# MiksuNy/rust_ray_tracing

Measured on AMD Instinct MI355X. Metric: Mray/s at 1920x1080, 8 spp, Sponza BVH; 1/2/4/8-GPU scaling + % HBM roofline, higher is better.
Workload: dtype f32

## Files before the change

include/mipt_diag.h:

```cpp
#ifndef MIPT_DIAG_H
#define MIPT_DIAG_H

#include <stdint.h>

#ifdef __cplusplus
extern "C" {
#endif

#if defined(__GNUC__)
#define MIPT_DIAG_API __attribute__((visibility("default")))
#else
#define MIPT_DIAG_API
#endif

MIPT_DIAG_API int mipt_debug_eval(int op, const float *a, const float *b, uint64_t n, float *out);

MIPT_DIAG_API int mipt_debug_eval_range(int op, uint32_t first_bits, uint64_t n, float y, float *out);

MIPT_DIAG_API int mipt_debug_wgsl(int op, const float *in, uint64_t n, const uint32_t *texels, uint32_t tex_w, uint32_t tex_h, float *out);

MIPT_DIAG_API int mipt_debug_divide(float *d_buf, uint64_t n_floats, float divisor, void *stream);
MIPT_DIAG_API int mipt_debug_popcount(const uint32_t *d_bitmap, uint64_t n_words, uint64_t *d_out, void *stream);

MIPT_DIAG_API const char *mipt_diag_last_error(void);

MIPT_DIAG_API int mipt_internal_pair_order(const void *nodes, uint32_t n_nodes, uint32_t *order_out, uint32_t cap, uint32_t *n_records_out);
MIPT_DIAG_API uint32_t mipt_internal_pair_order_top(void);
MIPT_DIAG_API int mipt_internal_tri_slots(const void *nodes, uint32_t n_nodes, uint32_t n_tris, uint32_t *slot_out, uint32_t *n_slots_out);

MIPT_DIAG_API int mipt_diag_scene_sizes(const void *scene, uint64_t out[2]);
MIPT_DIAG_API int mipt_diag_scene_read(const void *scene, int which, void *dst, uint64_t bytes);
MIPT_DIAG_API int mipt_diag_scene_hash(const void *scene, uint64_t out[2]);

MIPT_DIAG_API int mipt_diag_host_layout(const void *desc, uint8_t *geom_out, uint64_t geom_cap, uint8_t *attr_out, uint64_t attr_cap,
                                        uint64_t *sizes_out, uint32_t *info_out);

MIPT_DIAG_API int mipt_diag_hash_words(const void *words, uint64_t n_words, uint64_t *out);

MIPT_DIAG_API int mipt_diag_write_obj(const char *path, const void *tris, uint64_t n_tris, const char *mtllib, const char *const *material_names,
                                      uint32_t n_materials);

#ifdef __cplusplus
}
#endif
#endif
```

rust_ray_tracing_amd/_lib.py:

```python
from __future__ import annotations

import ctypes as C
import os

import numpy as np

_HERE = os.path.dirname(os.path.abspath(__file__))
LIB_PATH = os.environ.get("MIPT_LIB") or os.path.join(_HERE, "libmipt.so")

VERTEX = np.dtype([("position", "<f4", 3), ("tex_coord_x", "<f4"), ("normal", "<f4", 3), ("tex_coord_y", "<f4")])
TRIANGLE = np.dtype([("vertices", VERTEX, 3), ("material_id", "<u4"), ("_pad", "u1", 12)])
NODE = np.dtype([("bounds_min", "<f4", 3), ("first_tri_or_child", "<u4"), ("bounds_max", "<f4", 3), ("num_tris", "<u4")])
MATERIAL = np.dtype([
    ("base_color", "<f4", 3), ("transmission", "<f4"), ("specular_tint", "<f4", 3), ("ior", "<f4"),
    ("emission", "<f4", 3), ("roughness", "<f4"), ("metallic", "<f4"), ("transparency", "<f4"),
    ("base_color_tex_id", "<u4"), ("transparency_tex_id", "<u4"), ("roughness_tex_id", "<u4"),
    ("metallic_tex_id", "<u4"), ("emission_tex_id", "<u4"), ("normal_tex_id", "<u4")])
CAMERA = np.dtype([("look_at", "<f4", (4, 4)), ("position", "<f4", 3), ("_pad", "<f4")])
assert VERTEX.itemsize == 32 and TRIANGLE.itemsize == 112 and NODE.itemsize == 32
assert MATERIAL.itemsize == 80 and CAMERA.itemsize == 80

NO_TEXTURE = 0xFFFFFFFF

SEED_PIXEL_STREAM, SEED_PER_SAMPLE = 0, 1
# ... 240 lines not shown
    lib.mipt_query_closest_device.argtypes = [vp, vp, u64, qo, vp, vp, C.POINTER(MiptStats)]
    lib.mipt_query_closest_device.restype = C.c_int
    lib.mipt_query_occluded.argtypes = [vp, vp, u64, qo, vp, C.POINTER(MiptStats)]
    lib.mipt_query_occluded.restype = C.c_int
    lib.mipt_query_occluded_device.argtypes = [vp, vp, u64, qo, vp, vp, C.POINTER(MiptStats)]
    lib.mipt_query_occluded_device.restype = C.c_int
    fb = C.POINTER(MiptFeatureBuffers)
    lib.mipt_render_features.argtypes = [vp, vp, u32, C.POINTER(MiptOptions), fb, C.POINTER(MiptStats)]
    lib.mipt_render_features.restype = C.c_int
    lib.mipt_render_features_device.argtypes = [vp, vp, u32, C.POINTER(MiptOptions), fb, vp, C.POINTER(MiptStats)]
    lib.mipt_render_features_device.restype = C.c_int
    return lib


MULTITEST_LIB_PATH = os.path.join(_HERE, "libmipt_multitest.so")
_multitest = None


def load_multitest() -> C.CDLL:
    global _multitest
    if _multitest is not None:
        return _multitest
    load()
    if not os.path.exists(MULTITEST_LIB_PATH):
        raise ImportError(f"{MULTITEST_LIB_PATH} is missing: run __graft_entry__.build()")
    lib = _bind(C.CDLL(MULTITEST_LIB_PATH))
    lib.rccl_double_inject.argtypes = [C.c_int, C.c_int]
    lib.rccl_double_inject.restype = C.c_longlong
    _multitest = lib
    return lib


DIAG_LIB_PATH = os.path.join(_HERE, "libmipt_diag.so")
DIAG_EXPORTS = ["mipt_debug_eval", "mipt_debug_eval_range", "mipt_debug_wgsl", "mipt_debug_divide", "mipt_debug_popcount", "mipt_diag_last_error",
                "mipt_internal_pair_order", "mipt_internal_pair_order_top", "mipt_internal_tri_slots",
                "mipt_diag_scene_sizes", "mipt_diag_scene_read", "mipt_diag_scene_hash", "mipt_diag_write_obj", "mipt_diag_host_layout", "mipt_diag_hash_words"]
_diag = None


def load_diag() -> C.CDLL:
    global _diag
    if _diag is not None:
        return _diag
    load()
    if not os.path.exists(DIAG_LIB_PATH):
        raise ImportError(f"{DIAG_LIB_PATH} is missing: run __graft_entry__.build()")
    lib = C.CDLL(DIAG_LIB_PATH)
    vp = C.c_void_p
    lib.mipt_debug_eval.argtypes = [C.c_int, vp, vp, C.c_uint64, vp]
    lib.mipt_debug_eval.restype = C.c_int
    lib.mipt_debug_eval_range.argtypes = [C.c_int, C.c_uint32, C.c_uint64, C.c_float, vp]
    lib.mipt_debug_eval_range.restype = C.c_int
    lib.mipt_debug_wgsl.argtypes = [C.c_int, vp, C.c_uint64, vp, C.c_uint32, C.c_uint32, vp]
    lib.mipt_debug_wgsl.restype = C.c_int
    lib.mipt_debug_divide.argtypes = [vp, C.c_uint64, C.c_float, vp]
    lib.mipt_debug_divide.restype = C.c_int
    lib.mipt_debug_popcount.argtypes = [vp, C.c_uint64, vp, vp]
    lib.mipt_debug_popcount.restype = C.c_int
    lib.mipt_diag_last_error.argtypes = []
    lib.mipt_diag_last_error.restype = C.c_char_p
    u32p = C.POINTER(C.c_uint32)
    lib.mipt_internal_pair_order.argtypes = [vp, C.c_uint32, vp, C.c_uint32, u32p]
    lib.mipt_internal_pair_order.restype = C.c_int
    lib.mipt_internal_pair_order_top.argtypes = []
    lib.mipt_internal_pair_order_top.restype = C.c_uint32
    lib.mipt_internal_tri_slots.argtypes = [vp, C.c_uint32, C.c_uint32, vp, u32p]
    lib.mipt_internal_tri_slots.restype = C.c_int
    lib.mipt_diag_scene_sizes.argtypes = [vp, C.POINTER(C.c_uint64 * 2)]
    lib.mipt_diag_scene_sizes.restype = C.c_int
    lib.mipt_diag_scene_read.argtypes = [vp, C.c_int, vp, C.c_uint64]
    lib.mipt_diag_scene_read.restype = C.c_int
    lib.mipt_diag_scene_hash.argtypes = [vp, C.POINTER(C.c_uint64 * 2)]
    lib.mipt_diag_scene_hash.restype = C.c_int
    lib.mipt_diag_write_obj.argtypes = [C.c_char_p, vp, C.c_uint64, C.c_char_p, C.POINTER(C.c_char_p), C.c_uint32]
    lib.mipt_diag_write_obj.restype = C.c_int
    lib.mipt_diag_host_layout.argtypes = [vp, vp, C.c_uint64, vp, C.c_uint64, C.POINTER(C.c_uint64 * 2), C.POINTER(C.c_uint32 * 4)]
    lib.mipt_diag_host_layout.restype = C.c_int
    lib.mipt_diag_hash_words.argtypes = [vp, C.c_uint64, C.POINTER(C.c_uint64)]
    lib.mipt_diag_hash_words.restype = C.c_int
    _diag = lib
    return lib


class MiptError(RuntimeError):
    def __init__(self, code: int, where: str):
        self.code = code
        msg = load().mipt_last_error()
        super().__init__(f"{where} failed with status {code}: {msg.decode() if msg else ''}")


def check(code: int, where: str) -> None:
# ... 7 lines not shown
```

rust_ray_tracing_amd/csrc/mipt_api.cpp:

```cpp
#include "../../include/mipt.h"
#include "pt_kernel.h"
#include "mipt_scene.h"

#include <atomic>
#include <chrono>
#include <cmath>
#include <cstdarg>
#include <cstdio>
#include <cstdlib>
#include <cstring>
#include <exception>
#include <memory>
#include <mutex>
#include <new>
#include <string>
#include <thread>
#include <vector>

static_assert(sizeof(MiptVec3) == 12, "Vec3f");
static_assert(sizeof(MiptVertex) == 32, "Vertex");
static_assert(sizeof(MiptTriangle) == 112 && offsetof(MiptTriangle, material_id) == 96, "Triangle");
static_assert(sizeof(MiptNode) == 32 && offsetof(MiptNode, first_tri_or_child) == 12 &&
                  offsetof(MiptNode, bounds_max) == 16 && offsetof(MiptNode, num_tris) == 28, "Node");
static_assert(sizeof(MiptMaterial) == 80 && offsetof(MiptMaterial, ior) == 28 && offsetof(MiptMaterial, emission) == 32 &&
                  offsetof(MiptMaterial, roughness) == 44 && offsetof(MiptMaterial, base_color_tex_id) == 56, "Material");
static_assert(sizeof(MiptCamera) == 80 && offsetof(MiptCamera, position) == 64, "UniformCamera");
static_assert(sizeof(MiptStats) == 8 + 22 * 8 && sizeof(MiptOptions) == 64, "ABI struct sizes (tests/test_abi.py, rust_ray_tracing_amd/_lib.py)");
static_assert(sizeof(MiptSceneInfo) == 64, "MiptSceneInfo");
static_assert(sizeof(mipt::DevMaterial) == 64 && sizeof(mipt::DevMaterialFull) == 128, "device records");

namespace {

thread_local std::string g_err;

}

void mipt_internal_set_error(const char *msg) { g_err = msg ? msg : ""; }

void mipt::free_scene(MiptScene *s) {
    if (!s) return;
    (void)hipSetDevice(s->device);
    mipt::free_mesh(s);
    void *ptrs[] = {s->d_geom, s->d_tri_attr, s->d_mats, s->d_mats_full, s->d_texels, s->d_nodes, s->d_tri_order,
                    s->d_stats, s->d_ovf, s->d_hdr, s->d_rgba, s->d_touched, s->d_refit_plan, s->d_refit_pair, s->d_cams, s->d_qrays, s->d_qout};
    for (void *p : ptrs)
        if (p) (void)hipFree(p);
    if (s->ev0) (void)hipEventDestroy(s->ev0);
    if (s->ev1) (void)hipEventDestroy(s->ev1);
    delete s;
}

namespace {

using mipt::fail;
using mipt::free_scene;

double now_ms() { return std::chrono::duration<double, std::milli>(std::chrono::steady_clock::now().time_since_epoch()).count(); }

template <class T>
int upload(void **dst, const T *src, size_t count, size_t min_bytes = 16) {
    size_t bytes = count * sizeof(T);
    size_t alloc = bytes < min_bytes ? min_bytes : bytes;
    MIPT_HIP(hipMalloc(dst, alloc));
    if (bytes) MIPT_HIP(hipMemcpy(*dst, src, bytes, hipMemcpyHostToDevice));
    return MIPT_OK;
}
template <class T>
int upload(void **dst, const std::vector<T> &src, size_t min_bytes = 16) { return upload(dst, src.data(), src.size(), min_bytes); }

template <class F> void parallel_for(size_t n, F body) {
    unsigned t = std::thread::hardware_concurrency();
    if (t > 16u) t = 16u;
    if (t < 2u || n < (size_t)1 << 16) { body((size_t)0, n); return; }
    const size_t per = (n + t - 1) / t;
    std::vector<std::thread> th;
    size_t b = per;
    try {
// ... 423 lines not shown
    pr.samples_f = (float)opt->samples;
    pr.cull_scale = 1.0f + opt->cull_margin;
    pr.service_num = 3; pr.service_den = 8; pr.reverse_tiles = 0;
    for (int c = 0; c < 3; c++)
        for (int r = 0; r < 3; r++) pr.cam[c * 3 + r] = camera->look_at[c][r];
    pr.cam[9] = camera->position.x; pr.cam[10] = camera->position.y; pr.cam[11] = camera->position.z;
    pr.hdr = d_hdr_rgb;
    pr.stats = scene->d_stats;

    const bool count = (opt->flags & MIPT_FLAG_COUNT) != 0;
    const bool cull = opt->traversal == MIPT_TRAVERSAL_CULLED;
    const int occ = mipt::trace_blocks_per_cu(batch, count, cull, (int)opt->shading);
    int bpc = occ;
    {
        const long long fit = (long long)(pr.total_work / (unsigned long long)(1.25 * scene->n_cu * mipt::kBlockThreads));
        const int cap = (int)(fit < 2 ? 2 : fit);
        if (cap < bpc) bpc = cap;
    }
    pr.leaf_period = (pr.total_work >= 4ull * (unsigned long long)scene->n_cu * (unsigned long long)occ * mipt::kBlockThreads) ? 4u : 1u;
    pr.leaf_den = 4u;
    int grid = 0;
    if ((rc = mipt::traversal_grid(scene, bpc, pr.total_work, &grid))) return rc;
    pr.ovf = scene->d_ovf;

    const bool touched = count && (opt->flags & MIPT_FLAG_TOUCHED) != 0 && opt->shading == 0;
    const size_t geom_lines = ((size_t)scene->dev.geom_bytes + 127) / 128, attr_lines = (scene->n_tris + 1) / 2;
    const size_t geom_words = (geom_lines + 31) / 32, attr_words = (attr_lines + 31) / 32;
    pr.touched = nullptr; pr.touched_attr_base = (uint32_t)(geom_words * 32);
    if (touched) {
        if (!scene->d_touched) MIPT_HIP(hipMalloc((void **)&scene->d_touched, (geom_words + attr_words) * sizeof(uint32_t)));
        MIPT_HIP(hipMemsetAsync(scene->d_touched, 0, (geom_words + attr_words) * sizeof(uint32_t), stream));
        pr.touched = scene->d_touched;
    }
    mipt::DevBatch bt{};
    if (batch) {
        scene->h_cams.assign((size_t)n_views * 4, make_float4(0.0f, 0.0f, 0.0f, 0.0f));
        for (uint32_t v = 0; v < n_views; v++) {
            const MiptCamera &c = cameras[v];
            for (int col = 0; col < 3; col++) scene->h_cams[(size_t)v * 4 + col] = make_float4(c.look_at[col][0], c.look_at[col][1], c.look_at[col][2], 0.0f);
            scene->h_cams[(size_t)v * 4 + 3] = make_float4(c.position.x, c.position.y, c.position.z, 0.0f);
        }
        const size_t bytes = scene->h_cams.size() * sizeof(float4);
        if ((rc = mipt::grow_device_buffer((void **)&scene->d_cams, &scene->cams_bytes, bytes))) return rc;
        MIPT_HIP(hipMemcpyAsync(scene->d_cams, scene->h_cams.data(), bytes, hipMemcpyHostToDevice, stream));
        bt.cams = scene->d_cams;
        bt.view_pixels = opt->width * opt->height;
        bt.tiles_recip = 0xffffffffu / pr.n_local_tiles;
    }
    mipt::DevStats hs;
    float ms = 0.0f;
    rc = mipt::traversal_launch(
        scene, stream,
        [&]() -> int {
            MIPT_HIP(mipt::launch_trace(scene->dev, pr, batch ? &bt : nullptr, count, cull, (int)opt->shading, (int)grid, stream));
            return MIPT_OK;
        },
        [&]() -> int {
            if (touched) {
                MIPT_HIP(mipt::launch_popcount(scene->d_touched, geom_words, &scene->d_stats->touched_geom, stream));
                MIPT_HIP(mipt::launch_popcount(scene->d_touched + geom_words, attr_words, &scene->d_stats->touched_attr, stream));
            }
            if (d_rgba8) MIPT_HIP(mipt::launch_tonemap(d_hdr_rgb, (unsigned long long)opt->width * opt->height * n_views, 1.0f, d_rgba8, stream));
            return MIPT_OK;
        },
        hs, ms);
    if (rc && rc != MIPT_ERR_STACK) return rc;
    if (stats) {
        memset(stats, 0, sizeof *stats);
        stats->kernel_ms = ms;
        stats->rays = hs.rays; stats->inner_steps = hs.inner_steps; stats->tri_tests = hs.tri_tests;
        stats->hits = hs.hits; stats->texel_fetches = hs.texel_fetches; stats->stack_overflows = hs.stack_overflows;
        stats->tex_clamped = hs.tex_clamped; stats->max_stack = hs.max_stack; stats->pixels = hs.pixels;
        stats->diag[0] = hs.d_iters; stats->diag[1] = hs.d_inner_lanes; stats->diag[2] = hs.d_leaf_lanes;
        stats->diag[3] = hs.d_iters_inner; stats->diag[4] = hs.d_iters_leaf; stats->diag[5] = hs.d_services;
        stats->diag[6] = hs.d_service_lanes; stats->diag[7] = hs.d_cycles_service; stats->diag[8] = hs.d_cycles_total; stats->diag[9] = hs.d_cycles_mem; stats->diag[10] = hs.d_cycles_tail;
        stats->touched_lines[0] = hs.touched_geom; stats->touched_lines[1] = hs.touched_attr;
    }
    return rc;
}

int mipt::render_device_impl(MiptScene *scene, const MiptCamera *camera, const MiptOptions *opt,
                             float *d_hdr_rgb, uint8_t *d_rgba8, void *hip_stream, MiptStats *stats, bool pack_single) {
    return render_launch(scene, camera, 1u, false, opt, d_hdr_rgb, d_rgba8, hip_stream, stats, pack_single);
}

extern "C" {

int mipt_render_batch_device(MiptScene *scene, const MiptCamera *cameras, uint32_t n_views, const MiptOptions *opt,
                             float *d_hdr_rgb, uint8_t *d_rgba8, void *hip_stream, MiptStats *stats) {
    MIPT_NO_THROW(render_launch(scene, cameras, n_views, true, opt, d_hdr_rgb, d_rgba8, hip_stream, stats, false))
// ... 102 lines not shown
```

rust_ray_tracing_amd/csrc/mipt_diag.hip:

```cpp
#include "../../include/mipt_diag.h"
#include "pt_device_math.h"
#include "pt_device_wgsl.h"
#include "mipt_host_util.h"
#include "pt_kernel.h"

#include <stdio.h>

namespace {

thread_local char g_err[256] = "";

__global__ void debug_eval_kernel(int op, const float *__restrict__ a, const float *__restrict__ b, float b_scalar,
                                  unsigned long long n, float *__restrict__ out) {
    using namespace mipt;
    for (unsigned long long i = (unsigned long long)blockIdx.x * blockDim.x + threadIdx.x; i < n;
         i += (unsigned long long)gridDim.x * blockDim.x) {
        const float x = a[i], y = b ? b[i] : b_scalar;
        float r = 0.0f;
        switch (op) {
        case 0: r = gl_cosf(x); break;
        case 1: r = gl_log10f(x, GlTabGlobal()); break;
        case 2: r = gl_powf(x, y); break;
        case 3: r = x / y; break;
        case 4: r = __builtin_sqrtf(x); break;
        case 5: r = x * y; break;
        case 6: r = x + y; break;
        case 7: r = fminf(x, y); break;
        case 8: r = fmaxf(x, y); break;
        case 9: { uint32_t s = __float_as_uint(x); r = rand_f32(s); } break;
        case 10: { uint32_t s = __float_as_uint(x); r = rand_f32_nd(s, GlTabGlobal()); } break;
        case 11: { uint32_t s = __float_as_uint(x); V3 v = rand_in_unit_sphere(s, GlTabGlobal()); r = (y == 0.0f) ? v.x : (y == 1.0f ? v.y : v.z); } break;
        case 12: r = __uint_as_float(srgb_quantize(x)); break;
        case 13: r = x - truncf(x); break;
        case 14: r = fdiv_ray(x, y, 1.0f / y); break;
        case 15: r = u8_over_255(__float_as_uint(x)); break;
        case 16: r = gl_sinf(x); break;
        case 17: r = gl_expf(x); break;
// ... 111 lines not shown
        snprintf(g_err, sizeof g_err, "mipt_debug_wgsl: bad argument");
        return -1;
    }
    const uint64_t in_bytes = n * kWgslIn[op] * 4, out_bytes = n * kWgslOut[op] * 4;
    mipt::DevPtr<char> din, dtex, dout;
    hipError_t e;
    if ((e = din.alloc(in_bytes)) != hipSuccess) return fail(e, "hipMalloc");
    if ((e = dout.alloc(out_bytes)) != hipSuccess) return fail(e, "hipMalloc");
    if ((e = hipMemcpy(din, in, in_bytes, hipMemcpyHostToDevice)) != hipSuccess) return fail(e, "hipMemcpy");
    if (op == 0) {
        const uint64_t tex_bytes = (uint64_t)tex_w * tex_h * 4;
        if ((e = dtex.alloc(tex_bytes)) != hipSuccess) return fail(e, "hipMalloc");
        if ((e = hipMemcpy(dtex, texels, tex_bytes, hipMemcpyHostToDevice)) != hipSuccess) return fail(e, "hipMemcpy");
    }
    hipLaunchKernelGGL(debug_wgsl_kernel, dim3(1024), dim3(256), 0, nullptr, op, (const float *)din.get(), (unsigned long long)n,
                       (const uint32_t *)dtex.get(), tex_w, tex_h, (float *)dout.get(), kWgslIn[op], kWgslOut[op]);
    if ((e = hipGetLastError()) != hipSuccess) return fail(e, "launch");
    if ((e = hipMemcpy(out, dout, out_bytes, hipMemcpyDeviceToHost)) != hipSuccess) return fail(e, "hipMemcpy");
    return 0;
}

int mipt_debug_divide(float *d_buf, uint64_t n_floats, float divisor, void *stream) {
    if (!d_buf || n_floats == 0) { snprintf(g_err, sizeof g_err, "mipt_debug_divide: bad argument"); return -1; }
    const hipError_t e = mipt::launch_divide(d_buf, (unsigned long long)n_floats, divisor, (hipStream_t)stream);
    return e == hipSuccess ? 0 : fail(e, "launch_divide");
}

int mipt_debug_popcount(const uint32_t *d_bitmap, uint64_t n_words, uint64_t *d_out, void *stream) {
    if (!d_bitmap || !d_out || n_words == 0) { snprintf(g_err, sizeof g_err, "mipt_debug_popcount: bad argument"); return -1; }
    const hipError_t e = mipt::launch_popcount(d_bitmap, (unsigned long long)n_words, (unsigned long long *)d_out, (hipStream_t)stream);
    return e == hipSuccess ? 0 : fail(e, "launch_popcount");
}

const char *mipt_diag_last_error(void) { return g_err; }

}
```

rust_ray_tracing_amd/csrc/mipt_scene.h:

```cpp
#pragma once
#include "../../include/mipt.h"
#include "mipt_host_util.h"
#include "pt_kernel.h"

#include <stddef.h>

#include <memory>
#include <vector>

namespace mipt { struct SceneMesh; }

struct MiptScene {
    int device = 0;
    mipt::DevScene dev{};
    void *d_geom = nullptr, *d_tri_attr = nullptr, *d_mats = nullptr, *d_mats_full = nullptr, *d_texels = nullptr;
    size_t geom_alloc = 0, attr_bytes = 0, mats_bytes = 0, mats_full_bytes = 0, texel_bytes = 0;
    MiptNode *d_nodes = nullptr;
    uint32_t n_nodes = 0;
    uint32_t *d_tri_order = nullptr;
    MiptSceneInfo info{};
    mipt::DevStats *d_stats = nullptr;
    uint32_t *d_ovf = nullptr;
    size_t ovf_waves = 0;
    uint32_t *d_touched = nullptr;
    size_t n_tris = 0;
    float *d_hdr = nullptr;
    size_t hdr_bytes = 0;
    uint8_t *d_rgba = nullptr;
    size_t rgba_bytes = 0;
    float4 *d_cams = nullptr;
    size_t cams_bytes = 0;
    std::vector<float4> h_cams;
    void *d_qrays = nullptr, *d_qout = nullptr;
    size_t qrays_bytes = 0, qout_bytes = 0;
    hipEvent_t ev0 = nullptr, ev1 = nullptr;
    int n_cu = 0;
    uint32_t max_leaf = 0;
    uint32_t *d_refit_plan = nullptr, *d_refit_pair = nullptr;
    std::vector<uint32_t> refit_level_off;
    mipt::SceneMesh *mesh = nullptr;
};

namespace mipt {

void free_scene(MiptScene *s);
struct SceneDeleter { void operator()(MiptScene *s) const { free_scene(s); } };
using ScenePtr = std::unique_ptr<MiptScene, SceneDeleter>;
void free_mesh(MiptScene *s);
int scene_finish_workspace(MiptScene *s);
int scene_clone_to(const MiptScene *src, int device, MiptScene **out);
int scene_clone_many(const MiptScene *src, const int *device_ids, int n_dev, MiptScene **outs);

struct MaterialTables {
    std::vector<DevMaterial> mats;
    std::vector<DevMaterialFull> mats_full;
    std::vector<uint32_t> texels;
    std::vector<uint32_t> tex_offset;
    uint64_t n_texels = 0;
};
int build_material_tables(const MiptSceneDesc *desc, MaterialTables *out, bool gather_texels = true);
int upload_material_tables(MiptScene *s, const MaterialTables &t);

struct ResidentBvh {
    DevPtr<MiptNode> d_nodes;
    uint32_t n_nodes = 0;
// ... 57 lines not shown
```

rust_ray_tracing_amd/csrc/pt_kernel.h:

```cpp
#pragma once
#include <hip/hip_runtime.h>
#include <stdint.h>

namespace mipt {

struct DevMaterial {
    float base[3]; uint32_t base_off;
    float emis[3]; uint32_t emis_off;
    uint32_t base_w, base_h, emis_w, emis_h;
    uint32_t pad[4];
};

struct DevMaterialFull {
    float base[3]; float transmission;
    float emission[3]; float ior;
    float roughness, metallic, transparency, pad0;
    uint32_t tex[6][3];
    uint32_t pad1[2];
};

struct DevScene {
    const float4 *pairs;
    const float4 *tri_pos;
    uint32_t tri_off_bytes, geom_bytes;
// ... 2 lines not shown
    const DevMaterial *mats;
    const DevMaterialFull *mats_full;
    const uint32_t *texels;
    uint32_t n_pairs, n_tris, n_mats, n_texs;
    uint32_t root_a, root_n;
};

struct DevStats {
    unsigned long long queue;
    unsigned long long rays, inner_steps, tri_tests, hits, texel_fetches;
    unsigned long long stack_overflows, tex_clamped, max_stack, pixels;
    unsigned long long d_iters, d_inner_lanes, d_leaf_lanes, d_iters_inner, d_iters_leaf, d_services, d_service_lanes;
    unsigned long long d_cycles_service, d_cycles_total, d_cycles_mem, d_cycles_tail;
    unsigned long long touched_geom, touched_attr;
};

struct DevParams {
    uint32_t width, height, samples, max_depth;
    uint32_t seed_mode, sample_begin, sum_only, packed;
    uint32_t accumulate, pad1;
    uint32_t tile_rank, tile_world, tiles_x, tiles_y;
    uint32_t n_local_tiles, pad0;
    unsigned long long total_work;
    float aspect;
    float samples_f;
    float cull_scale;
    uint32_t reverse_tiles;
    uint32_t service_num, service_den;
    uint32_t leaf_period, leaf_den;
    float cam[12];
    float *hdr;
    uint32_t *ovf;
    DevStats *stats;
    uint32_t *touched;
    uint32_t touched_attr_base;
};

struct DevBatch {
    const float4 *cams;
    uint32_t view_pixels;
    uint32_t tiles_recip;
};

constexpr int kStackLds = 16;
constexpr int kStackOvf = 48;
constexpr int kWavesPerBlock = 4;
constexpr uint32_t kTriPosStride = 64;
constexpr int kBlockThreads = 64 * kWavesPerBlock;
constexpr uint32_t kMaxTris = 1u << 25;
constexpr uint32_t kMaxPairs = 1u << 24;

hipError_t launch_trace(const DevScene &sc, const DevParams &pr, const DevBatch *batch, bool count, bool cull, int shading,
                        int grid_blocks, hipStream_t stream);
int trace_blocks_per_cu(bool batch, bool count, bool cull, int shading);
hipError_t launch_unpack_tiles(const float *packed_all, uint32_t width, uint32_t height,
                               uint32_t tile_world, float *hdr, hipStream_t stream);
hipError_t launch_tonemap(const float *hdr, unsigned long long n_pixels, float divisor,
                          uint8_t *rgba8, hipStream_t stream);

struct DevQuery {
    const float4 *rays;
    void *out;
    const uint32_t *tri_order;
    unsigned long long n_rays;
    float cull_scale;
    uint32_t *ovf;
    DevStats *stats;
};
hipError_t launch_ray_query(const DevScene &sc, const DevQuery &q, bool count, bool cull, bool anyhit, int grid_blocks, hipStream_t stream);
int query_blocks_per_cu(bool count, bool cull, bool anyhit);

struct DevFeatures {
    const float4 *cams;
    float *depth; uint32_t *prim; uint32_t *material; float *position; float *uv; float *normal; float *albedo; float *emission;
    const uint32_t *tri_order;
    uint32_t width, height, samples, seed_mode;
    uint32_t sample_begin;
    uint32_t tiles_x, n_tiles;
    uint32_t tiles_recip;
    uint32_t view_pixels;
    unsigned long long total_work;
    float aspect;
    float samples_f;
    float cull_scale;
    uint32_t *ovf;
    DevStats *stats;
};
hipError_t launch_first_hit(const DevScene &sc, const DevFeatures &f, bool count, bool cull, int grid_blocks, hipStream_t stream);
int first_hit_blocks_per_cu(bool count, bool cull);

hipError_t launch_popcount(const uint32_t *bitmap, unsigned long long n_words, unsigned long long *out, hipStream_t stream);
hipError_t launch_divide(float *hdr, unsigned long long n_floats, float divisor, hipStream_t stream);
hipError_t launch_postprocess(const float *hdr, unsigned long long n_pixels, float divisor, uint16_t *rgba16,
                              hipStream_t stream);

}
```

rust_ray_tracing_amd/csrc/pt_kernel.hip:

```cpp
#include "pt_kernel.h"
#include "pt_device_math.h"
#include "pt_device_wgsl.h"
#include "pt_traverse.h"

namespace mipt {

namespace {

#ifndef MIPT_DIAG_STAMPS
#define MIPT_DIAG_STAMPS 0
#endif
constexpr bool DIAG_STAMPS = MIPT_DIAG_STAMPS != 0;

enum : uint32_t {
    ST_T = 0,
    ST_S = 1,
    ST_G = 2,
    ST_P = 3,
    ST_X = 4
};

__device__ __forceinline__ float min3_abs(float a, float b, float c) { float r; asm("v_min3_f32 %0, |%1|, |%2|, |%3|" : "=v"(r) : "v"(a), "v"(b), "v"(c)); return r; }

__device__ __forceinline__ void mark_line(uint32_t *bitmap, uint32_t line) {
// ... 210 lines not shown
                }
            }
            if (SHADING == 0) {
                float *dr = s_draw[wib];
                const unsigned long long m_sc = __ballot(scatter);
                const uint32_t n_items = 3u * (uint32_t)__popcll(m_sc);
                if (n_items != 0u) {
                    const uint32_t base = 6u * lane_rank(m_sc);
                    if (scatter) {
#pragma unroll
                        for (int k = 0; k < 6; k++) dr[base + k] = rand_f32(rng);
                    }
                    __builtin_amdgcn_fence(__ATOMIC_ACQ_REL, "wavefront");
                    __builtin_amdgcn_wave_barrier();
                    for (uint32_t item = lane; item < n_items; item += 64u) {
                        const float2 uu = *reinterpret_cast<const float2 *>(dr + 2u * item);
                        dr[2u * item] = rand_f32_nd_eval(uu.x, uu.y, (const double *)s_logtab);
                    }
                    __builtin_amdgcn_fence(__ATOMIC_ACQ_REL, "wavefront");
                    __builtin_amdgcn_wave_barrier();
                    if (scatter) {
                        const V3 rs = normalized(mk(dr[base], dr[base + 2u], dr[base + 4u]));
                        const V3 point = o + d * best_t;
                        const V3 new_dir = normalized(sc_normal + rs);
                        o = point + new_dir * 0.0001f;
                        d = new_dir;
                        bounces += 1;
                        path_done = !(bounces < pr.max_depth);
                    }
                }
            }
            if (state == ST_S) {
                if (path_done) {
                    const V3 res = (bounces == 0u) ? incoming : incoming / (float)bounces;
                    final_color = final_color + res;
                    sample += 1;
                    if (sample < pr.samples) {
                        state = ST_G;
                    } else {
                        if (!pr.sum_only) final_color = final_color / pr.samples_f;
                        float *dst = pr.hdr + (BATCH ? (size_t)view * bt.view_pixels + pix : (size_t)slot) * 3;
                        if (pr.accumulate) {
                            final_color = mk(dst[0] + final_color.x, dst[1] + final_color.y, dst[2] + final_color.z);
                        }
                        dst[0] = final_color.x; dst[1] = final_color.y; dst[2] = final_color.z;
                        c_pixels++;
                        state = ST_P;
                    }
                } else {
                    state = ST_T;
                    start_ray = true;
                }
            }
            {
                const unsigned long long m_p = __ballot(state == ST_P);
                if (m_p != 0ull) {
                    unsigned long long base = 0;
                    const uint32_t leader = (uint32_t)__ffsll((long long)m_p) - 1u;
                    if (lane == leader) base = atomicAdd(&pr.stats->queue, (unsigned long long)__popcll(m_p));
                    base = __shfl(base, (int)leader);
                    if (state == ST_P) {
                        const unsigned long long wi = base + lane_rank(m_p);
                        if (wi >= pr.total_work) {
                            state = ST_X;
                            if (COUNT && g_t_first_x == 0) g_t_first_x = clock64();
                        } else {
                            uint32_t lt = (uint32_t)(wi >> 6);
                            const uint32_t p = (uint32_t)wi & 63u;
                            if (BATCH) {
                                const uint32_t n = pr.n_local_tiles;
                                uint32_t q = __umulhi(lt, bt.tiles_recip), r = lt - q * n;
                                if (r >= n) { q += 1u; r -= n; }
                                if (r >= n) { q += 1u; r -= n; }
                                view = q; lt = r;
                            }
                            const uint32_t lt_o = pr.reverse_tiles ? (pr.n_local_tiles - 1u - lt) : lt;
                            const uint32_t gt = lt_o * pr.tile_world + pr.tile_rank;
                            const uint32_t px = (gt % pr.tiles_x) * 8u + (p & 7u);
                            const uint32_t py = (gt / pr.tiles_x) * 8u + (p >> 3);
                            if (px < pr.width && py < pr.height) {
                                pix = py * pr.width + px;
                                if (!BATCH) slot = pr.packed ? (lt_o * 64u + p) : pix;
                                rng = 987612486u * (pix + 87636354u);
                                const uint32_t y = pr.height - py;
                                screen_x = ((((float)px / (float)pr.width) * 2.0f) - 1.0f) * pr.aspect;
                                screen_y = (((float)y / (float)pr.height) * 2.0f) - 1.0f;
                                final_color = mk(0.0f, 0.0f, 0.0f);
                                sample = 0;
                                state = ST_G;
                            }
                        }
                    }
                }
            }
            if (state == ST_G) {
                if (SHADING == 1 || pr.seed_mode != 0u) {
                    const uint32_t px = pix % pr.width, py = pix / pr.width;
                    rng = (pr.sample_begin + sample) * 6023u + (757283u * px + 872653746u * py);
                }
                const float jx = (rand_f32(rng) * 2.0f - 1.0f) * 0.0005f;
                const float jy = (rand_f32(rng) * 2.0f - 1.0f) * 0.0005f;
                const float rx = -screen_x + jx, ry = screen_y + jy, rz = 1.0f;
                if (BATCH) {
                    const float4 *cr = bt.cams + (size_t)view * 4;
                    const float4 c0 = cr[0], c1 = cr[1], c2 = cr[2], c3 = cr[3];
                    const V3 dir = mk(c0.x * rx + c1.x * ry + c2.x * rz,
                                      c0.y * rx + c1.y * ry + c2.y * rz,
                                      c0.z * rx + c1.z * ry + c2.z * rz);
                    d = normalized(dir);
                    o = mk(c3.x, c3.y, c3.z);
                } else {
                    const V3 dir = mk(pr.cam[0] * rx + pr.cam[3] * ry + pr.cam[6] * rz,
                                      pr.cam[1] * rx + pr.cam[4] * ry + pr.cam[7] * rz,
                                      pr.cam[2] * rx + pr.cam[5] * ry + pr.cam[8] * rz);
                    d = normalized(dir);
// ... 138 lines not shown
        }
        {
            const unsigned long long tx = __shfl(g_t_first_x, (int)(__ffsll((long long)__ballot(g_t_first_x != 0)) - 1));
            if (lane == 0 && tx != 0) atomicAdd(&pr.stats->d_cycles_tail, clock64() - tx);
        }
    }
    if (c_pixels) atomicAdd(&pr.stats->pixels, (unsigned long long)c_pixels);
}

template <bool COUNT, bool CULL, int SHADING>
__global__ MIPT_TRACE_BOUNDS(COUNT, CULL, SHADING) void pt_trace_kernel(DevScene sc, DevParams pr) {
    trace_body<COUNT, CULL, SHADING, false>(sc, pr, DevBatch{});
}
template <bool COUNT, bool CULL, int SHADING>
__global__ MIPT_TRACE_BOUNDS(COUNT, CULL, SHADING) void pt_trace_batch_kernel(DevScene sc, DevParams pr, DevBatch bt) {
    trace_body<COUNT, CULL, SHADING, true>(sc, pr, bt);
}

__global__ void unpack_tiles_kernel(const float *__restrict__ packed_all, uint32_t width, uint32_t height,
                                    uint32_t world, uint32_t tiles_x, uint32_t n_local_tiles, float *__restrict__ hdr) {
    const unsigned long long n = (unsigned long long)width * height;
    for (unsigned long long i = (unsigned long long)blockIdx.x * blockDim.x + threadIdx.x; i < n;
         i += (unsigned long long)gridDim.x * blockDim.x) {
        const uint32_t px = (uint32_t)(i % width), py = (uint32_t)(i / width);
        const uint32_t gt = (py >> 3) * tiles_x + (px >> 3);
        const uint32_t rank = gt % world, lt = gt / world;
        const unsigned long long src = ((unsigned long long)rank * n_local_tiles + lt) * 64ull + ((py & 7u) * 8u + (px & 7u));
        hdr[i * 3 + 0] = packed_all[src * 3 + 0];
        hdr[i * 3 + 1] = packed_all[src * 3 + 1];
        hdr[i * 3 + 2] = packed_all[src * 3 + 2];
    }
}

__global__ void popcount_kernel(const uint32_t *__restrict__ bitmap, unsigned long long n_words, unsigned long long *out) {
    unsigned long long c = 0;
    for (unsigned long long i = (unsigned long long)blockIdx.x * blockDim.x + threadIdx.x; i < n_words;
         i += (unsigned long long)gridDim.x * blockDim.x)
        c += (unsigned long long)__popc(bitmap[i]);
    for (int o = 32; o > 0; o >>= 1) c += __shfl_down(c, o);
    if ((threadIdx.x & 63u) == 0u && c) atomicAdd(out, c);
}
hipError_t launch_popcount(const uint32_t *bitmap, unsigned long long n_words, unsigned long long *out, hipStream_t stream) {
    hipLaunchKernelGGL(popcount_kernel, dim3(1024), dim3(256), 0, stream, bitmap, n_words, out);
    return hipGetLastError();
}

__global__ void divide_kernel(float *__restrict__ hdr, unsigned long long n_floats, float divisor) {
    for (unsigned long long i = (unsigned long long)blockIdx.x * blockDim.x + threadIdx.x; i < n_floats;
         i += (unsigned long long)gridDim.x * blockDim.x)
        hdr[i] = hdr[i] / divisor;
}
hipError_t launch_divide(float *hdr, unsigned long long n_floats, float divisor, hipStream_t stream) {
    hipLaunchKernelGGL(divide_kernel, dim3(2048), dim3(256), 0, stream, hdr, n_floats, divisor);
    return hipGetLastError();
}

__global__ void tonemap_kernel(const float *__restrict__ hdr, unsigned long long n, float divisor, uint32_t *__restrict__ rgba8) {
    for (unsigned long long i = (unsigned long long)blockIdx.x * blockDim.x + threadIdx.x; i < n;
         i += (unsigned long long)gridDim.x * blockDim.x) {
        float r = hdr[i * 3 + 0], g = hdr[i * 3 + 1], b = hdr[i * 3 + 2];
        if (divisor != 1.0f) { r = r / divisor; g = g / divisor; b = b / divisor; }
        rgba8[i] = srgb_quantize(r) | (srgb_quantize(g) << 8) | (srgb_quantize(b) << 16) | 0xff000000u;
    }
}

__device__ __forceinline__ float pp_channel(float c) {
// ... 86 lines not shown
```

Baseline: 2627.

## Schedule tiles longest-first using per-tile bounce cost from previous frame

Adds per-tile cost accumulation (bounces per path) during tracing and a single-block counting-sort kernel that orders tiles by descending cost. The next frame with the same camera and settings hands out tiles in that order, a longest-processing-time-first schedule meant to reduce tail imbalance in the persistent work queue. It adds an atomic per finished path, a small sort kernel per frame and a memset. The order only applies when the camera and key match the previous frame, so the first frame pays the overhead without any benefit.

```diff
diff --git a/include/mipt_diag.h b/include/mipt_diag.h
--- a/include/mipt_diag.h
+++ b/include/mipt_diag.h
@@ -22,6 +22,9 @@
 MIPT_DIAG_API int mipt_debug_divide(float *d_buf, uint64_t n_floats, float divisor, void *stream);
 MIPT_DIAG_API int mipt_debug_popcount(const uint32_t *d_bitmap, uint64_t n_words, uint64_t *d_out, void *stream);
 
+MIPT_DIAG_API int mipt_debug_tile_order(const uint32_t *cost, uint32_t n_tiles, uint32_t samples, uint32_t *order_out);
+MIPT_DIAG_API int mipt_diag_scene_tile_order(const void *scene, uint32_t *cost_out, uint32_t *order_out, uint32_t cap, uint32_t info_out[3]);
+
 MIPT_DIAG_API const char *mipt_diag_last_error(void);
 
 MIPT_DIAG_API int mipt_internal_pair_order(const void *nodes, uint32_t n_nodes, uint32_t *order_out, uint32_t cap, uint32_t *n_records_out);
diff --git a/rust_ray_tracing_amd/_lib.py b/rust_ray_tracing_amd/_lib.py
--- a/rust_ray_tracing_amd/_lib.py
+++ b/rust_ray_tracing_amd/_lib.py
@@ -296,7 +296,7 @@
 
 
 DIAG_LIB_PATH = os.path.join(_HERE, "libmipt_diag.so")
-DIAG_EXPORTS = ["mipt_debug_eval", "mipt_debug_eval_range", "mipt_debug_wgsl", "mipt_debug_divide", "mipt_debug_popcount", "mipt_diag_last_error",
+DIAG_EXPORTS = ["mipt_debug_eval", "mipt_debug_eval_range", "mipt_debug_wgsl", "mipt_debug_divide", "mipt_debug_popcount", "mipt_debug_tile_order", "mipt_diag_scene_tile_order", "mipt_diag_last_error",
                 "mipt_internal_pair_order", "mipt_internal_pair_order_top", "mipt_internal_tri_slots",
                 "mipt_diag_scene_sizes", "mipt_diag_scene_read", "mipt_diag_scene_hash", "mipt_diag_write_obj", "mipt_diag_host_layout", "mipt_diag_hash_words"]
 _diag = None
@@ -321,6 +321,10 @@
     lib.mipt_debug_divide.restype = C.c_int
     lib.mipt_debug_popcount.argtypes = [vp, C.c_uint64, vp, vp]
     lib.mipt_debug_popcount.restype = C.c_int
+    lib.mipt_debug_tile_order.argtypes = [vp, C.c_uint32, C.c_uint32, vp]
+    lib.mipt_debug_tile_order.restype = C.c_int
+    lib.mipt_diag_scene_tile_order.argtypes = [vp, vp, vp, C.c_uint32, C.POINTER(C.c_uint32 * 3)]
+    lib.mipt_diag_scene_tile_order.restype = C.c_int
     lib.mipt_diag_last_error.argtypes = []
     lib.mipt_diag_last_error.restype = C.c_char_p
     u32p = C.POINTER(C.c_uint32)
diff --git a/rust_ray_tracing_amd/csrc/mipt_api.cpp b/rust_ray_tracing_amd/csrc/mipt_api.cpp
--- a/rust_ray_tracing_amd/csrc/mipt_api.cpp
+++ b/rust_ray_tracing_amd/csrc/mipt_api.cpp
@@ -42,7 +42,8 @@
     (void)hipSetDevice(s->device);
     mipt::free_mesh(s);
     void *ptrs[] = {s->d_geom, s->d_tri_attr, s->d_mats, s->d_mats_full, s->d_texels, s->d_nodes, s->d_tri_order,
-                    s->d_stats, s->d_ovf, s->d_hdr, s->d_rgba, s->d_touched, s->d_refit_plan, s->d_refit_pair, s->d_cams, s->d_qrays, s->d_qout};
+                    s->d_stats, s->d_ovf, s->d_hdr, s->d_rgba, s->d_touched, s->d_refit_plan, s->d_refit_pair, s->d_cams, s->d_qrays, s->d_qout,
+                    s->d_tile_cost, s->d_tile_order};
     for (void *p : ptrs)
         if (p) (void)hipFree(p);
     if (s->ev0) (void)hipEventDestroy(s->ev0);
@@ -532,6 +533,24 @@
         MIPT_HIP(hipMemsetAsync(scene->d_touched, 0, (geom_words + attr_words) * sizeof(uint32_t), stream));
         pr.touched = scene->d_touched;
     }
+    const bool order_on = !count && !batch && opt->shading == MIPT_SHADING_CPU && !(opt->flags & MIPT_FLAG_ACCUM) && pr.n_local_tiles != 0u;
+    pr.tile_order = nullptr; pr.tile_cost = nullptr;
+    if (order_on) {
+        const uint32_t key[7] = {opt->width, opt->height, world, opt->tile_rank, pr.n_local_tiles, pr.seed_mode, opt->samples};
+        const size_t bytes = (size_t)pr.n_local_tiles * sizeof(uint32_t);
+        if (scene->tile_cost_bytes < bytes || scene->tile_order_bytes < bytes || memcmp(key, scene->tile_key, sizeof key) != 0 ||
+            memcmp(pr.cam, scene->tile_cam, sizeof pr.cam) != 0)
+            scene->tile_order_valid = false;
+        if ((rc = mipt::grow_device_buffer((void **)&scene->d_tile_cost, &scene->tile_cost_bytes, bytes))) return rc;
+        if ((rc = mipt::grow_device_buffer((void **)&scene->d_tile_order, &scene->tile_order_bytes, bytes))) return rc;
+        memcpy(scene->tile_key, key, sizeof key);
+        memcpy(scene->tile_cam, pr.cam, sizeof pr.cam);
+        MIPT_HIP(hipMemsetAsync(scene->d_tile_cost, 0, bytes, stream));
+        pr.tile_cost = scene->d_tile_cost;
+        pr.tile_order = scene->tile_order_valid ? scene->d_tile_order : nullptr;
+        scene->tile_order_used = scene->tile_order_valid;
+        scene->tile_order_valid = false;
+    }
     mipt::DevBatch bt{};
     if (batch) {
         scene->h_cams.assign((size_t)n_views * 4, make_float4(0.0f, 0.0f, 0.0f, 0.0f));
@@ -556,6 +575,10 @@
             return MIPT_OK;
         },
         [&]() -> int {
+            if (order_on) {
+                MIPT_HIP(mipt::launch_tile_order(scene->d_tile_cost, pr.n_local_tiles, opt->samples, scene->d_tile_order, stream));
+                scene->tile_order_valid = true;
+            }
             if (touched) {
                 MIPT_HIP(mipt::launch_popcount(scene->d_touched, geom_words, &scene->d_stats->touched_geom, stream));
                 MIPT_HIP(mipt::launch_popcount(scene->d_touched + geom_words, attr_words, &scene->d_stats->touched_attr, stream));
diff --git a/rust_ray_tracing_amd/csrc/mipt_diag.hip b/rust_ray_tracing_amd/csrc/mipt_diag.hip
--- a/rust_ray_tracing_amd/csrc/mipt_diag.hip
+++ b/rust_ray_tracing_amd/csrc/mipt_diag.hip
@@ -3,6 +3,7 @@
 #include "pt_device_wgsl.h"
 #include "mipt_host_util.h"
 #include "pt_kernel.h"
+#include "mipt_scene.h"
 
 #include <stdio.h>
 
@@ -180,6 +181,33 @@
     return e == hipSuccess ? 0 : fail(e, "launch_popcount");
 }
 
+int mipt_debug_tile_order(const uint32_t *cost, uint32_t n_tiles, uint32_t samples, uint32_t *order_out) {
+    if (!cost || !order_out || n_tiles == 0 || samples == 0) { snprintf(g_err, sizeof g_err, "mipt_debug_tile_order: bad argument"); return -1; }
+    mipt::DevPtr<uint32_t> dcost, dorder;
+    hipError_t e;
+    if ((e = dcost.alloc(n_tiles)) != hipSuccess) return fail(e, "hipMalloc");
+    if ((e = dorder.alloc(n_tiles)) != hipSuccess) return fail(e, "hipMalloc");
+    if ((e = hipMemcpy(dcost, cost, (size_t)n_tiles * 4, hipMemcpyHostToDevice)) != hipSuccess) return fail(e, "hipMemcpy");
+    if ((e = hipMemset(dorder, 0xff, (size_t)n_tiles * 4)) != hipSuccess) return fail(e, "hipMemset");
+    if ((e = mipt::launch_tile_order(dcost, n_tiles, samples, dorder, nullptr)) != hipSuccess) return fail(e, "launch_tile_order");
+    if ((e = hipMemcpy(order_out, dorder, (size_t)n_tiles * 4, hipMemcpyDeviceToHost)) != hipSuccess) return fail(e, "hipMemcpy");
+    return 0;
+}
+
+int mipt_diag_scene_tile_order(const void *scene, uint32_t *cost_out, uint32_t *order_out, uint32_t cap, uint32_t info_out[3]) {
+    const MiptScene *s = (const MiptScene *)scene;
+    if (!s || !info_out) { snprintf(g_err, sizeof g_err, "mipt_diag_scene_tile_order: bad argument"); return -1; }
+    const uint32_t n = s->tile_order_valid ? s->tile_key[4] : 0u;
+    info_out[0] = n; info_out[1] = s->tile_order_valid ? 1u : 0u; info_out[2] = s->tile_order_used ? 1u : 0u;
+    if (n == 0u || !cost_out || !order_out) return 0;
+    if (cap < n) { snprintf(g_err, sizeof g_err, "mipt_diag_scene_tile_order: cap %u < %u tiles", cap, n); return -1; }
+    hipError_t e;
+    if ((e = hipSetDevice(s->device)) != hipSuccess) return fail(e, "hipSetDevice");
+    if ((e = hipMemcpy(cost_out, s->d_tile_cost, (size_t)n * 4, hipMemcpyDeviceToHost)) != hipSuccess) return fail(e, "hipMemcpy");
+    if ((e = hipMemcpy(order_out, s->d_tile_order, (size_t)n * 4, hipMemcpyDeviceToHost)) != hipSuccess) return fail(e, "hipMemcpy");
+    return 0;
+}
+
 const char *mipt_diag_last_error(void) { return g_err; }
 
 }
diff --git a/rust_ray_tracing_amd/csrc/mipt_scene.h b/rust_ray_tracing_amd/csrc/mipt_scene.h
--- a/rust_ray_tracing_amd/csrc/mipt_scene.h
+++ b/rust_ray_tracing_amd/csrc/mipt_scene.h
@@ -31,6 +31,12 @@
     float4 *d_cams = nullptr;
     size_t cams_bytes = 0;
     std::vector<float4> h_cams;
+    uint32_t *d_tile_cost = nullptr, *d_tile_order = nullptr;
+    size_t tile_cost_bytes = 0, tile_order_bytes = 0;
+    uint32_t tile_key[7] = {0, 0, 0, 0, 0, 0, 0};
+    float tile_cam[12] = {0};
+    bool tile_order_valid = false;
+    bool tile_order_used = false;
     void *d_qrays = nullptr, *d_qout = nullptr;
     size_t qrays_bytes = 0, qout_bytes = 0;
     hipEvent_t ev0 = nullptr, ev1 = nullptr;
diff --git a/rust_ray_tracing_amd/csrc/pt_kernel.h b/rust_ray_tracing_amd/csrc/pt_kernel.h
--- a/rust_ray_tracing_amd/csrc/pt_kernel.h
+++ b/rust_ray_tracing_amd/csrc/pt_kernel.h
@@ -58,6 +58,8 @@
     float *hdr;
     uint32_t *ovf;
     DevStats *stats;
+    const uint32_t *tile_order;
+    uint32_t *tile_cost;
     uint32_t *touched;
     uint32_t touched_attr_base;
 };
@@ -115,6 +117,7 @@
 hipError_t launch_first_hit(const DevScene &sc, const DevFeatures &f, bool count, bool cull, int grid_blocks, hipStream_t stream);
 int first_hit_blocks_per_cu(bool count, bool cull);
 
+hipError_t launch_tile_order(const uint32_t *cost, uint32_t n_tiles, uint32_t samples, uint32_t *order, hipStream_t stream);
 hipError_t launch_popcount(const uint32_t *bitmap, unsigned long long n_words, unsigned long long *out, hipStream_t stream);
 hipError_t launch_divide(float *hdr, unsigned long long n_floats, float divisor, hipStream_t stream);
 hipError_t launch_postprocess(const float *hdr, unsigned long long n_pixels, float divisor, uint16_t *rgba16,
diff --git a/rust_ray_tracing_amd/csrc/pt_kernel.hip b/rust_ray_tracing_amd/csrc/pt_kernel.hip
--- a/rust_ray_tracing_amd/csrc/pt_kernel.hip
+++ b/rust_ray_tracing_amd/csrc/pt_kernel.hip
@@ -266,6 +266,7 @@
             }
             if (state == ST_S) {
                 if (path_done) {
+                    if (!BATCH && pr.tile_cost) atomicAdd(&pr.tile_cost[slot >> 6], bounces + ((best_tri == kNoTri) ? 1u : 0u));
                     const V3 res = (bounces == 0u) ? incoming : incoming / (float)bounces;
                     final_color = final_color + res;
                     sample += 1;
@@ -273,7 +274,7 @@
                         state = ST_G;
                     } else {
                         if (!pr.sum_only) final_color = final_color / pr.samples_f;
-                        float *dst = pr.hdr + (BATCH ? (size_t)view * bt.view_pixels + pix : (size_t)slot) * 3;
+                        float *dst = pr.hdr + (BATCH ? (size_t)view * bt.view_pixels + pix : (size_t)(pr.packed ? slot : pix)) * 3;
                         if (pr.accumulate) {
                             final_color = mk(dst[0] + final_color.x, dst[1] + final_color.y, dst[2] + final_color.z);
                         }
@@ -308,13 +309,13 @@
                                 if (r >= n) { q += 1u; r -= n; }
                                 view = q; lt = r;
                             }
-                            const uint32_t lt_o = pr.reverse_tiles ? (pr.n_local_tiles - 1u - lt) : lt;
+                            const uint32_t lt_o = (!BATCH && pr.tile_order) ? pr.tile_order[lt] : (pr.reverse_tiles ? (pr.n_local_tiles - 1u - lt) : lt);
                             const uint32_t gt = lt_o * pr.tile_world + pr.tile_rank;
                             const uint32_t px = (gt % pr.tiles_x) * 8u + (p & 7u);
                             const uint32_t py = (gt / pr.tiles_x) * 8u + (p >> 3);
                             if (px < pr.width && py < pr.height) {
                                 pix = py * pr.width + px;
-                                if (!BATCH) slot = pr.packed ? (lt_o * 64u + p) : pix;
+                                if (!BATCH) slot = lt_o * 64u + p;
                                 rng = 987612486u * (pix + 87636354u);
                                 const uint32_t y = pr.height - py;
                                 screen_x = ((((float)px / (float)pr.width) * 2.0f) - 1.0f) * pr.aspect;
@@ -519,6 +520,62 @@
     }
 }
 
+constexpr uint32_t kOrderBuckets = 1024, kOrderWaves = 8, kOrderThreads = 64 * kOrderWaves;
+__device__ __forceinline__ uint32_t tile_bucket(uint32_t cost, float scale) {
+    const float b = (float)cost * scale;
+    return (kOrderBuckets - 1u) - (b < (float)(kOrderBuckets - 1u) ? (uint32_t)b : (kOrderBuckets - 1u));
+}
+__global__ __launch_bounds__(kOrderThreads) void tile_order_kernel(const uint32_t *__restrict__ cost, uint32_t n, float scale, uint32_t *__restrict__ order) {
+    __shared__ uint32_t s_cnt[kOrderWaves][kOrderBuckets];
+    __shared__ uint32_t s_scan[kOrderThreads];
+    const uint32_t t = threadIdx.x, lane = t & 63u, w = t >> 6;
+    for (uint32_t i = t; i < kOrderWaves * kOrderBuckets; i += kOrderThreads) (&s_cnt[0][0])[i] = 0u;
+    __syncthreads();
+    const uint32_t per = ((n + kOrderThreads - 1u) / kOrderThreads) * 64u;
+    const unsigned long long lo64 = (unsigned long long)w * per;
+    const uint32_t lo = lo64 < n ? (uint32_t)lo64 : n, hi = (lo64 + per < n) ? (uint32_t)(lo64 + per) : n;
+    for (uint32_t i = lo + lane; i < hi; i += 64u) atomicAdd(&s_cnt[w][tile_bucket(cost[i], scale)], 1u);
+    __syncthreads();
+    uint32_t tot = 0u;
+    for (uint32_t k = 0; k < 2u; k++)
+        for (uint32_t ww = 0; ww < kOrderWaves; ww++) { const uint32_t c = s_cnt[ww][2u * t + k]; s_cnt[ww][2u * t + k] = tot; tot += c; }
+    s_scan[t] = tot;
+    __syncthreads();
+    for (uint32_t o = 1u; o < kOrderThreads; o <<= 1) {
+        const uint32_t y = t >= o ? s_scan[t - o] : 0u;
+        __syncthreads();
+        s_scan[t] += y;
+        __syncthreads();
+    }
+    const uint32_t base = s_scan[t] - tot;
+    for (uint32_t k = 0; k < 2u; k++)
+        for (uint32_t ww = 0; ww < kOrderWaves; ww++) s_cnt[ww][2u * t + k] += base;
+    __syncthreads();
+    for (uint32_t i0 = lo; i0 < hi; i0 += 64u) {
+        const uint32_t i = i0 + lane;
+        const bool valid = i < hi;
+        const uint32_t b = valid ? tile_bucket(cost[i], scale) : 0u;
+        unsigned long long peers = __ballot(valid);
+        for (uint32_t k = 0; k < 10u; k++) {
+            const bool bit = ((b >> k) & 1u) != 0u;
+            const unsigned long long m = __ballot(valid && bit);
+            peers &= bit ? m : ~m;
+        }
+        if (valid) {
+            const uint32_t rank = lane_rank(peers);
+            const uint32_t at = s_cnt[w][b];
+            if (rank == 0u) s_cnt[w][b] = at + (uint32_t)__popcll(peers);
+            order[at + rank] = i;
+        }
+        __builtin_amdgcn_fence(__ATOMIC_ACQ_REL, "wavefront");
+        __builtin_amdgcn_wave_barrier();
+    }
+}
+hipError_t launch_tile_order(const uint32_t *cost, uint32_t n_tiles, uint32_t samples, uint32_t *order, hipStream_t stream) {
+    hipLaunchKernelGGL(tile_order_kernel, dim3(1), dim3(kOrderThreads), 0, stream, cost, n_tiles, 16.0f / (64.0f * (float)samples), order);
+    return hipGetLastError();
+}
+
 __global__ void popcount_kernel(const uint32_t *__restrict__ bitmap, unsigned long long n_words, unsigned long long *out) {
     unsigned long long c = 0;
     for (unsigned long long i = (unsigned long long)blockIdx.x * blockDim.x + threadIdx.x; i < n_words;
```

Measured after the change: 2685, median of 6. 2.2% higher.
